# klkuhlm/unconfined

Hardware: AMD Instinct MI355X
Metric: (t,r) drawdown points/sec, Neuman-1974 1024x256 sweep; max |rel err| vs CPU ref (higher is better)
Workload: dtype f64

## Files before the change

unconfined_amd/csrc/ucf_device.h:

```cpp

#include "ucf_math.h"
#include "ucf_plan.h"
#include <cstdlib>

namespace UCF_NS {

using namespace ucfm;

#define UCF_STR_(x) #x
#define UCF_STR(x) UCF_STR_(x)
#define UCF_PI 3.14159265358979323846
#define UCF_EPS 2.220446049250313e-16

UCF_DEV double shfl_down1(double v) { return __shfl_down(v, 1, 64); }
UCF_DEV double shift_down1(double x)
{
    const int lo = __double2loint(x), hi = __double2hiint(x);
    const int l2 = __builtin_amdgcn_update_dpp(lo, lo, 0x130, 0xf, 0xf, false);
    const int h2 = __builtin_amdgcn_update_dpp(hi, hi, 0x130, 0xf, 0xf, false);
    return __hiloint2double(h2, l2);
}
UCF_DEV cplx shfl_down1(cplx v) { return cmake(shift_down1(v.re), shift_down1(v.im)); }
UCF_DEV cplx bcast0(cplx v) { return cmake(__shfl(v.re, 0, 64), __shfl(v.im, 0, 64)); }
UCF_DEV double wave_max(double v)
// ... 1245 lines not shown
__global__ void __launch_bounds__(UCF_WAVE * UCF_IWPB, WAVES)
integrate_kernel(const ucf_dev_params P0, int npts, int per_point, int nr, int nsv, int svmin,
                 const double* __restrict__ tDv, const double* __restrict__ rDv, const int* __restrict__ svv,
                 const double2* __restrict__ tab, int nt, int ir0, double2* __restrict__ state, int* __restrict__ ndone,
                 int* __restrict__ todo, const ucf_dev_params* __restrict__ Pv, int ppp, int pbase, int lsplit,
                 const double2* __restrict__ ltab, int nrows, int nheadw, int nworkw, int* __restrict__ wcount)
{
    extern __shared__ lds_c lds[];
#ifdef UCF_K1_ASSUME
    const ucf_dev_params& P = P0;
    UCF_K1_ASSUME
#endif
    const int lane = threadIdx.x & (UCF_WAVE - 1), wv = __builtin_amdgcn_readfirstlane(threadIdx.x / UCF_WAVE);
    constexpr int EF = (FAMILY == 5) ? 1 : FAMILY;
    constexpr bool ZPAIR = FOLD && EF == 2 && NZC == 1;
    const int nz = NZC ? NZC : P0.nz, R = P0.R, nacc = P0.nacc, N = P0.N, ngl = P0.ngl;
    __builtin_assume(nz >= 1 && R >= 1 && nacc >= 1 && ngl >= 1);
    const int nabs = N + nacc * ngl;
    {
        const double2* __restrict__ gt = (const double2*)P0.sc_tab;
        for (int k = threadIdx.x; k < UCF_SC_ENTRIES; k += UCF_WAVE * UCF_IWPB) lds[k] = gt[k];
    }
    __syncthreads();
    const lds_c* sct = lds;
    const int lslots = (NZC ? R : R + 1) * nz;
    lds_c* const wlds = lds + UCF_SC_ENTRIES + (size_t)wv * lslots * UCF_WAVE;
    lds_c* accTS = wlds;
    lds_c* accCur = wlds + (size_t)R * nz * UCF_WAVE;
    int ustat = blockIdx.x * UCF_IWPB + wv - gridDim.x * UCF_IWPB;
    auto next_unit = [&]() {
        if (!wcount) return ustat += gridDim.x * UCF_IWPB;
        int u = 0;
        if (lane == 0) u = __hip_atomic_fetch_add(wcount, 1, __ATOMIC_RELAXED, __HIP_MEMORY_SCOPE_AGENT);
        return __builtin_amdgcn_readfirstlane(u);
    };
    for (int wi = next_unit(); wi < nworkw; wi = next_unit()) {
        const bool tail = wi >= nheadw;
        const int ls = tail ? (lsplit >> 8) : (lsplit & 255), nsplit = 1 << ls;
        const int wj = tail ? wi - nheadw : wi;
        const int pt = (tail ? (nheadw >> (lsplit & 255)) : 0) + (wj >> ls), sub = wj & (nsplit - 1);
        auto part_bound = [&](int k) {
            if (k <= 0) return 0;
            if (k >= nsplit) return nabs;
            int j = (k * nabs / nsplit - N + ngl / 2) / ngl;
            j = j < 0 ? 0 : (j > nacc ? nacc : j);
            return N + j * ngl;
        };
        const int n0 = part_bound(sub), n1 = part_bound(sub + 1);
        if (n1 <= n0 && sub != 0) continue;
#ifdef UCF_TIMELINE
        const unsigned long long tl_t0 = __builtin_amdgcn_s_memtime();
#endif
        const work_item W = decode_item<LAYOUT>(P0, pt, lane, per_point, nr, nt, ir0, npts);
        const ucf_dev_params& P = item_params<MULTI>(P0, Pv, (LAYOUT == 3 ? W.plan * ppp : W.pidx) + pbase, ppp);
        bool need_lay1 = false, need_lay3 = false, need_lay12 = false;
        for (int z = 0; z < nz; z++) { need_lay1 |= (P.zLay[z] == 1); need_lay3 |= (P.zLay[z] == 3); need_lay12 |= (P.zLay[z] != 3); }
        const double tD = tDv[W.it], rD = rDv[W.ir];
        const int sv = (LAYOUT == 1) ? svmin : svv[W.it];
        const double2* __restrict__ row = tab + (size_t)(per_point ? W.pidx : (W.ir * nsv + (sv - svmin))) * nabs;
        const double tee = 2.0 * tD;
        const double sigma = P.alpha - P.logtol / (2.0 * tee);
        const cplx p = cmake(sigma, UCF_PI * W.mlap / tee);
        const double2 ltv = ltab[(size_t)(W.mlap < P0.np ? W.mlap : P0.np - 1) * nrows + W.it];
        const cplx lt = cmake(ltv.x, ltv.y);
        const lane_consts LC = make_lane_consts(P, p, lt);
        auto lt_again = [&]() {
            int it = W.it;
            asm volatile("" : "+v"(it));
            const double2 v = ltab[(size_t)(W.mlap < P0.np ? W.mlap : P0.np - 1) * nrows + it];
            return cmake(v.x, v.y);
        };
        double2* __restrict__ sti = state + (size_t)pt * state_slots(P0) * UCF_WAVE;
        double2* __restrict__ areas = sti + (size_t)(R + 1) * nz * UCF_WAVE;
        for (int s = 0; s < lslots; s++) lds_st(wlds, s, lane, cmake(0.0, 0.0));
        fast_common F;
        sc_ctx_init(F.sc, sct, UCF_KV(FAMILY, FOLD));
        const bool lane_ok = FAMILY != 2 || (fabs(LC.xifac.re) + fabs(LC.xifac.im) < 1.0e90);
        const int nlim = (__builtin_amdgcn_ballot_w64(!lane_ok) == 0) ? n1 : n0;

        int n = n0;
        double2 aa = row[n0 < nabs ? n0 : 0];
        int m = 0, jj = n0 > N ? (n0 - N) / ngl : 0;
        cplx acc0 = cmake(0.0, 0.0), acc1 = cmake(0.0, 0.0);
        if constexpr (ZPAIR) {
            int stopped = 0;
            const int nts = nlim < N ? nlim : N;
            for (; n < nts; n++) {
                const double2 nxt = row[n + 1 < nabs ? n + 1 : n];
                F.sc.salt = n;
                if (!fast_eta_wave<EF, true>(P, LC, aa.x, F)) { stopped = 1; break; }
                const cplx val = rscale(aa.y, fast_sample_zpair<!MULTI>(P, LC, F));
                const int n1 = n + 1;
                int tz = __builtin_ctz(n1);
                if (tz > R - 1) tz = R - 1;
                for (int sh = 0; sh <= tz; sh++) {
                    const int j = R - sh;
                    const double wl = P.ts_w[(size_t)(j - 1) * N + ((n1 >> sh) - 1)];
                    lds_st(accTS, j - 1, lane, cadd(lds_ld(accTS, j - 1, lane), rscale(wl, val)));
                }
                aa = nxt;
            }
            if (!stopped) for (; n < nlim; n++) {
                const double2 nxt = row[n + 1 < nabs ? n + 1 : n];
                F.sc.salt = n;
                if (!fast_eta_wave<EF, true>(P, LC, aa.x, F)) break;
                const cplx fz = fast_sample_zpair<!MULTI>(P, LC, F);
                acc0 = cmake(__builtin_fma(fz.re, aa.y, acc0.re), __builtin_fma(fz.im, aa.y, acc0.im));
                if (++m == ngl) {
                    const double lob = P.j0z[sv + jj - 1] / rD;
                    const double hib = P.j0z[sv + jj] / rD;
                    const double hw = (hib - lob) / 2.0;
                    const cplx ar = cmul(rscale(hw, acc0), lt_again());
                    areas[(size_t)jj * UCF_WAVE + lane] = make_double2(ar.re, ar.im);
                    acc0 = cmake(0.0, 0.0);
                    m = 0;
                    jj++;
                }
                aa = nxt;
            }
        } else
        for (; n < nlim; n++) {
            const double2 nxt = row[n + 1 < nabs ? n + 1 : n];
            const bool ts = n < N;
            F.sc.salt = n;
            if (!fast_eta_wave<EF, ZPAIR>(P, LC, aa.x, F)) break;
            if constexpr (!ZPAIR) fast_common_terms<EF, FOLD, LAY3, LAY1, NOFOLD, ZPAIR>(P, LC, aa.x, need_lay1, F, need_lay3, need_lay12);
            const int n1 = n + 1;
            int tz = __builtin_ctz(n1);
            if (tz > R - 1) tz = R - 1;
            for (int z = 0; z < nz; z++) {
                cplx fz;
                if constexpr (ZPAIR) fz = fast_sample_zpair<!MULTI>(P, LC, F);
                else fz = fast_sample_z<EF, FOLD, LAY3, LAY1, NOFOLD, ZPAIR>(P, F, z);
                if (ts) {
                    const cplx val = rscale(aa.y, fz);
                    for (int sh = 0; sh <= tz; sh++) {
                        const int j = R - sh;
                        const double wl = P.ts_w[(size_t)(j - 1) * N + ((n1 >> sh) - 1)];
                        const int slot = (j - 1) * nz + z;
                        lds_st(accTS, slot, lane, cadd(lds_ld(accTS, slot, lane), rscale(wl, val)));
                    }
                } else if (nz == 1 || (NZC == 2 && z == 0)) {
                    acc0 = cmake(__builtin_fma(fz.re, aa.y, acc0.re), __builtin_fma(fz.im, aa.y, acc0.im));
                } else if (NZC == 2) {
                    acc1 = cmake(__builtin_fma(fz.re, aa.y, acc1.re), __builtin_fma(fz.im, aa.y, acc1.im));
                } else {
                    const cplx a1 = lds_ld(accCur, z, lane);
                    lds_st(accCur, z, lane, cmake(__builtin_fma(fz.re, aa.y, a1.re), __builtin_fma(fz.im, aa.y, a1.im)));
                }
            }
            if (!ts && ++m == ngl) {
                const double lob = P.j0z[sv + jj - 1] / rD;
                const double hib = P.j0z[sv + jj] / rD;
                const double hw = (hib - lob) / 2.0;
                for (int z = 0; z < nz; z++) {
                    const cplx run = (nz == 1 || (NZC == 2 && z == 0)) ? acc0 : (NZC == 2 ? acc1 : lds_ld(accCur, z, lane));
                    const cplx ar = cmul(rscale(hw, run), lt);
                    areas[(size_t)(jj * nz + z) * UCF_WAVE + lane] = make_double2(ar.re, ar.im);
                    if (nz != 1 && NZC != 2) lds_st(accCur, z, lane, cmake(0.0, 0.0));
                }
                acc0 = acc1 = cmake(0.0, 0.0);
                m = 0;
                jj++;
            }
            aa = nxt;
        }
        if (sub == 0) {
            const cplx lte = ZPAIR ? lt_again() : lt;
            for (int s = 0; s < R * nz; s++) {
                const cplx v = cmul(lds_ld(wlds, s, lane), lte);
                sti[(size_t)s * UCF_WAVE + lane] = make_double2(v.re, v.im);
            }
            for (int s = R * nz; s < (R + 1) * nz; s++) sti[(size_t)s * UCF_WAVE + lane] = make_double2(0.0, 0.0);
        }
#ifdef UCF_TIMELINE
        if (sub == 0) {
            const unsigned long long tl_t1 = __builtin_amdgcn_s_memtime();
            const unsigned hwid = __builtin_amdgcn_s_getreg(63492);
            if (lane == 0) sti[(size_t)(R * nz) * UCF_WAVE + 0] = make_double2(__longlong_as_double((long long)tl_t0), __longlong_as_double((long long)tl_t1));
            if (lane == 1) sti[(size_t)(R * nz) * UCF_WAVE + 1] = make_double2((double)hwid, (double)__builtin_amdgcn_s_getreg(63508));
        }
#endif
        if (n < n1 && lane == 0) {
            const int nrep = (n < N) ? n : n - m;
            if (atomicMin(&ndone[pt], nrep) == nabs) todo[1 + atomicAdd(&todo[0], 1)] = pt;
        }
    }
}

#endif

template <int FAMILY, int LAYOUT>
__global__ void __launch_bounds__(UCF_WAVE, 3)
integrate_generic_kernel(const ucf_dev_params P, int npts, int per_point, int nr, int nsv, int svmin,
                         const double* __restrict__ tDv, const double* __restrict__ rDv, const int* __restrict__ svv,
                         const double2* __restrict__ tab, int nt, int ir0, double2* __restrict__ state, int* __restrict__ ndone)
{
    extern __shared__ lds_c lds[];
    const int lane = threadIdx.x;
    const int nz = P.nz, R = P.R, nacc = P.nacc, N = P.N, ngl = P.ngl;
    const int nabs = N + nacc * ngl;
    lds_c* accTS = lds;
    lds_c* accCur = lds + (size_t)R * nz * UCF_WAVE;
    lds_c* fdbuf = accCur + (size_t)nz * UCF_WAVE;
    bool need_lay1 = false;
    for (int z = 0; z < nz; z++) need_lay1 |= (P.zLay[z] == 1);
    for (int pt = blockIdx.x; pt < npts; pt += gridDim.x) {
        const work_item W = decode_item<LAYOUT>(P, pt, lane, per_point, nr, nt, ir0, npts);
        const double tD = tDv[W.it], rD = rDv[W.ir];
        const int sv = (LAYOUT == 1) ? svmin : svv[W.it];
        const double2* __restrict__ row = tab + (size_t)(per_point ? W.pidx : (W.ir * nsv + (sv - svmin))) * nabs;
        const double tee = 2.0 * tD;
        const double sigma = P.alpha - P.logtol / (2.0 * tee);
        const cplx p = cmake(sigma, UCF_PI * W.mlap / tee);
        const cplx lt = lap_time(P, p);
// ... 888 lines not shown
```

unconfined_amd/csrc/ucf_fastpath.h:

```cpp
#pragma once

namespace UCF_NS {

#define UCF_UNIFORM_BLOCK() asm volatile("" ::: "memory")
#define UCF_UNIFORM_BLOCK_F(FAMILY) do { if constexpr ((FAMILY) != 4) UCF_UNIFORM_BLOCK(); } while (0)

struct fprim {
    double ch, sh, ei, sn, cs;
};

template <bool POS>
UCF_DEV fprim prim_from_e(double x, double ax, double e, double ei, double y, const sc_ctx& sc)
{
    const int salt = sc.salt;
    fprim f;
    f.ei = ei;
    const double he = 0.5 * e;
    f.ch = __builtin_fma(0.5, ei, he);
    double s;
    if (ax < 0.35) {
        const double x2 = ax * ax;
        double pl = addk(mulk(x2, UCF_KHERE(1.0 / 6227020800.0, salt)), UCF_KHERE(1.0 / 39916800.0, salt));
        pl = fmak(pl, x2, UCF_KHERE(1.0 / 362880.0, salt));
        pl = fmak(pl, x2, UCF_KHERE(1.0 / 5040.0, salt));
        pl = fmak(pl, x2, UCF_KHERE(1.0 / 120.0, salt));
        pl = fmak(pl, x2, UCF_KHERE(1.0 / 6.0, salt));
        s = __builtin_fma(ax * x2, pl, ax);
    } else {
        s = __builtin_fma(-0.5, ei, he);
    }
    f.sh = POS ? s : copysign(s, x);
    sincos_tab_(y, sc, &f.sn, &f.cs);
    return f;
}
template <bool POS = false>
UCF_DEV fprim prim(double x, double y, const sc_ctx& sc)
{
    const double ax = POS ? x : fabs(x);
    const double e = exp_tab_(ax, sc);
    return prim_from_e<POS>(x, ax, e, fast_rcp(e), y, sc);
}
UCF_DEV void prim_pair(double x, double y, double zD, double xcap, const sc_ctx& sc, fprim* f, fprim* fz)
{
    const double xc = fmin(x, xcap);
    const double xz = xc * zD;
    const double e = exp_tab_(xc, sc), ez = exp_tab_(xz, sc);
    const double r = fast_rcp(e * ez);
    *f = prim_from_e<true>(xc, xc, e, r * ez, y, sc);
    *fz = prim_from_e<true>(xz, xz, ez, r * e, y * zD, sc);
}
template <bool UNI>
UCF_DEV void prim_pair_min(double x, double y, double zD, double xcap, const sc_ctx& sc, fprim* f, fprim* fz)
{
    double xc;
    if constexpr (UNI) asm("v_min_f64 %0, %1, %2" : "=v"(xc) : "v"(x), "s"(xcap));
    else xc = fmin(x, xcap);
    const double xz = xc * zD;
    const double e = exp_tab_(xc, sc), ez = exp_tab_(xz, sc);
    const double r = fast_rcp(e * ez);
    *f = prim_from_e<true>(xc, xc, e, r * ez, y, sc);
    *fz = prim_from_e<true>(xz, xz, ez, r * e, y * zD, sc);
}
UCF_DEV fprim prim_difference(const fprim& a, const fprim& b)
{
    fprim f;
    const double e = (a.ch + a.sh) * b.ei;
    const double ei = a.ei * (b.ch + b.sh);
    f.ei = ei;
    f.ch = 0.5 * (e + ei);
    f.sh = 0.5 * (e - ei);
    f.sn = __builtin_fma(a.sn, b.cs, -(a.cs * b.sn));
    f.cs = __builtin_fma(a.cs, b.cs, a.sn * b.sn);
    return f;
}
UCF_DEV cplx pcosh(const fprim& f) { return cmake(f.ch * f.cs, f.sh * f.sn); }
UCF_DEV cplx psinh(const fprim& f) { return cmake(f.sh * f.cs, f.ch * f.sn); }
UCF_DEV cplx pexpneg(const fprim& f) { return cmake(f.ei * f.cs, -(f.ei * f.sn)); }

UCF_DEV cplx expneg_direct(double x, double y, const sc_ctx& sc)
{
    const double ei = exp_tab_(-x, sc);
    double sn, cs;
    sincos_tab_(y, sc, &sn, &cs);
    return cmake(ei * cs, -(ei * sn));
}

UCF_DEV cplx cfma(cplx a, cplx b, cplx c)
{
    return cmake(__builtin_fma(a.re, b.re, __builtin_fma(-a.im, b.im, c.re)), __builtin_fma(a.re, b.im, __builtin_fma(a.im, b.re, c.im)));
}
UCF_DEV cplx cfnma(cplx a, cplx b, cplx c)
{
    return cmake(__builtin_fma(-a.re, b.re, __builtin_fma(a.im, b.im, c.re)), __builtin_fma(-a.re, b.im, __builtin_fma(-a.im, b.re, c.im)));
}
UCF_DEV cplx cinv_plain(cplx z)
{
    const double r = fast_rcp(z.re * z.re + z.im * z.im);
    return cmake(z.re * r, -(z.im * r));
}
UCF_DEV cplx cinv_scaled(cplx z)
{
    const double m = fmax(fabs(z.re), fabs(z.im));
    const int il = __builtin_amdgcn_frexp_exp(m) - 1;
    const double c = ldexp(z.re, -il), d = ldexp(z.im, -il);
    const double r = fast_rcp(c * c + d * d);
    return cmake(ldexp(c * r, -il), ldexp(-(d * r), -il));
}

UCF_DEV cplx cinv_auto(cplx z)
{
    const double m = fmax(fabs(z.re), fabs(z.im));
    if (__builtin_amdgcn_ballot_w64(!(m < 1.0e150 && m > 1.0e-150)) == 0) return cinv_plain(z);
    return cinv_scaled(z);
}

struct lane_consts {
    cplx p, lt, xifac;
    cplx fdB1;
    cplx mnpv;
};

UCF_DEV lane_consts make_lane_consts(const ucf_dev_params& P, cplx p, cplx lt)
{
    lane_consts L;
    L.p = p;
    L.lt = lt;
    cplx xf = rscale(P.alphaD, cinv_plain(p));
    if (P.model == 3) {
        cplx sum = cmake(0.0, 0.0);
        for (int j = 0; j < P.MoenchM; j++) sum = cadd(sum, cinv_plain(radd(1.0, cscale(p, P.MoenchInvGamma[j]))));
        xf = cmul(cscale(xf, (double)P.MoenchM), cinv_plain(sum));
    }
    L.xifac = xf;
    L.fdB1 = cscale(cscale(cscale(p, P.fd_beta0), P.fd_expmb2), P.inv_kappa);
    L.mnpv = radd(1.0, cscale(p, P.mn_vartheta * P.mn_c3));
    return L;
}

struct fast_common {
    sc_ctx sc;
    cplx th, eta, ff1, ff2, inv_she, she, che, top, g3, inv_den, ex1;
    cplx chz0;
    fprim p1;
    int have_p1;
    cplx mn_uod;
#ifdef UCF_SINGLE_RCP
    cplx q, den;
#endif
    cplx fd_s1;
    cplx top3, fd_s13;
    bool small_eta, fd_use, fd_use3;
    int any_small, any_large;
};

template <int FAMILY>
UCF_DEV double fast_scale(const ucf_dev_params& P)
{
    if (FAMILY == 0 || FAMILY == 3) return 2.0;
    if (FAMILY == 5) return P.inv_bD;
    return (FAMILY == 2 && P.model == 4) ? 2.0 : 2.0 * P.inv_bD;
}

template <int FAMILY, bool PAIR = false>
UCF_DEV bool fast_eta(const ucf_dev_params& P, const lane_consts& L, double a, fast_common& S)
{
    const double a2 = a * a;
    const cplx q = caddr(L.p, a2);
#ifdef UCF_SINGLE_RCP
    S.q = q;
#endif
    double mq = 0.0;
    if (PAIR && FAMILY != 0) {
        double r;
        rsq_pair(q.re * q.re + q.im * q.im, &mq, &r);
        S.th = cmake(q.re * r, -(q.im * r));
    } else {
        const double r = fast_rcp(q.re * q.re + q.im * q.im);
        S.th = cmake(q.re * r, -(q.im * r));
    }
    if (FAMILY == 0) return q.re > 0.0;
    {
        const double qr = q.re * P.inv_kappa, qi = q.im * P.inv_kappa;
        double r, hr;
        const double d = PAIR ? mq * P.inv_kappa : sqrt_only(__builtin_fma(qr, qr, qi * qi));
        sqrt_hrsqrt(0.5 * (d + qr), &r, &hr);
        S.eta = cmake(r, qi * hr);
    }
    return (S.eta.re <= P.fast_eta_max) & (q.re > 0.0) & (fabs(S.eta.im) < P.fast_im_max);
}
template <int FAMILY, bool PAIR = false>
UCF_DEV bool fast_eta_wave(const ucf_dev_params& P, const lane_consts& L, double a, fast_common& S)
{
    (void)fast_eta<FAMILY, PAIR>(P, L, a, S);
    const cplx q = caddr(L.p, a * a);
    unsigned long long bad = __builtin_amdgcn_ballot_w64(!(q.re > 0.0));
    if (FAMILY != 0) {
        bad |= __builtin_amdgcn_ballot_w64(!(S.eta.re <= P.fast_eta_max));
        bad |= __builtin_amdgcn_ballot_w64(!(fabs(S.eta.im) < P.fast_im_max));
    }
    return bad == 0;
}

template <int FAMILY, bool FOLD = false, bool LAY3 = true, bool LAY1 = true, bool NOFOLD = false, bool ZPAIR = false>
UCF_DEV void fast_common_terms(const ucf_dev_params& P, const lane_consts& L, double a, bool need_lay1_in, fast_common& S,
                               bool need_lay3_in = false, bool need_lay12 = true)
{
    static_assert(!ZPAIR || (FOLD && FAMILY == 2), "ZPAIR: folded water-table kernels only");
    const double a2 = a * a;
    if (FAMILY == 0) return;
    if (FAMILY == 3) {
        const fprim p1 = prim<true>(S.eta.re, S.eta.im, S.sc);
        S.che = pcosh(p1);
        S.she = psinh(p1);
        const double wr = __builtin_fma(a2, P.mn_c3, L.mnpv.re), wi = L.mnpv.im;
        double vr, hr;
        sqrt_hrsqrt(0.5 * (sqrt_only(__builtin_fma(wr, wr, wi * wi)) + wr), &vr, &hr);
        const cplx u = cmake(P.mn_u0 * (1.0 - vr), -(P.mn_u0 * (wi * hr)));
        const cplx Delta0 = cfnma(u, S.che, cmul(S.eta, S.she));
        S.mn_uod = cmul(u, cinv_auto(Delta0));
        return;
    }
    const bool hantush = NOFOLD || !(FAMILY == 2 && P.model == 4);
    const bool z1 = FOLD || (!NOFOLD && P.fold_dD != 0), z2 = FOLD || (!NOFOLD && P.fold_lD1 != 0);
    const bool need_lay1 = (FOLD || !LAY1) ? false : need_lay1_in;
    const bool need_lay3 = (FOLD || !LAY3) ? false : need_lay3_in;
    S.small_eta = (FAMILY != 2) || (S.eta.re < P.maxexp);
    S.any_small = ((FAMILY != 2) || (__builtin_amdgcn_ballot_w64(S.small_eta) != 0)) ? 1 : 0;
    S.any_large = ((FAMILY == 2) && (__builtin_amdgcn_ballot_w64(!S.small_eta) != 0)) ? 1 : 0;
    const bool need_p1 = (hantush && (!(z1 && z2) || need_lay1)) || FAMILY == 4 || (FAMILY == 2 && S.any_small);
    S.have_p1 = (need_p1 && !z2) ? 1 : 0;
    fprim p1;
    if (ZPAIR && need_p1) {
        fprim pz;
        prim_pair(S.eta.re, S.eta.im, P.zD[0], P.maxexp, S.sc, &p1, &pz);
        S.chz0 = pcosh(pz);
        S.che = pcosh(p1);
        S.she = psinh(p1);
        S.ex1 = cmake(0.0, 0.0);
    } else if (need_p1) {
        p1 = prim<true>(S.eta.re, S.eta.im, S.sc);
        if (!z2) S.p1 = p1;
        S.che = pcosh(p1);
        S.she = psinh(p1);
        if (need_lay1) S.ex1 = pexpneg(p1);
        else S.ex1 = cmake(0.0, 0.0);
    } else {
        S.che = S.she = S.ex1 = cmake(0.0, 0.0);
    }
    if (hantush) {
        fprim pd;
        if (!z1) { pd = prim<true>(S.eta.re * P.dD, S.eta.im * P.dD, S.sc); S.ff1 = psinh(pd); }
        else S.ff1 = cmake(0.0, 0.0);
        fprim pl;
        if (!z2) { pl = prim<true>(S.eta.re * P.lD1, S.eta.im * P.lD1, S.sc); S.ff2 = psinh(pl); }
        else S.ff2 = cmake(0.0, 0.0);
        if (!(z1 && z2) || need_lay1) S.inv_she = cinv_auto(S.she);
        if (need_lay1) {
            const cplx exl = z2 ? cmake(1.0, 0.0) : pexpneg(pl);
            S.g3 = csub(exl, cmul(cadd(S.ff1, cmul(S.ex1, S.ff2)), S.inv_she));
        }
        if (FAMILY != 1) {
            S.top = S.top3 = S.th;
            if (!(z1 && z2)) {
                if (need_lay12) {
                    cplx g1;
                    if (z1) g1 = cmake(1.0, 0.0);
                    else if (P.share_g1top == 1) g1 = pcosh(pd);
                    else if (P.share_g1top == 2) g1 = csub(pcosh(pd), cmul(rscale(P.g1_delta, S.eta), S.ff1));
                    else { const double c = P.dD1 - 1.0; g1 = pcosh(prim(S.eta.re * c, S.eta.im * c, S.sc)); }
                    const cplx udp = csub(g1, cmul(cadd(cmul(S.ff1, S.che), S.ff2), S.inv_she));
                    S.top = cmul(udp, S.th);
                }
                if (need_lay3) {
                    cplx sd1 = S.she;
                    if (!z1) {
                        const double x1 = S.eta.re * P.dD1;
                        if (__builtin_amdgcn_ballot_w64(!(x1 >= 1.0)) == 0) sd1 = psinh(prim_difference(p1, pd));
                        else sd1 = psinh(prim(x1, S.eta.im * P.dD1, S.sc));
                    }
                    const cplx udp = cmul(z2 ? sd1 : csub(sd1, S.ff2), S.inv_she);
                    S.top3 = cmul(udp, S.th);
// ... 75 lines not shown
    cplx chz = cmake(1.0, 0.0);
    fprim pz;
    if (ZPAIR) { if (need_chz) chz = S.chz0; }
    else if (need_chz) { pz = prim<true>(S.eta.re * zD, S.eta.im * zD, S.sc); chz = pcosh(pz); }
    *chz_out = chz;
    cplx udp;
    if (lay == 1) {
        udp = cmul(S.g3, chz);
    } else {
        cplx g2 = cmake(0.0, 0.0);
        const bool need_1z = !z2;
        fprim p1z;
        if (z2 && FAMILY == 2 && S.any_large) {
            const double c = 1.0 - zD;
            *exz_out = expneg_direct(S.eta.re * c, S.eta.im * c, S.sc);
            UCF_UNIFORM_BLOCK_F(FAMILY);
        }
        if (need_1z) {
            if (need_chz && S.have_p1 && zD >= 0.0 && zD <= 1.0) p1z = prim_difference(S.p1, pz);
            else
            { const double c = 1.0 - zD; p1z = prim(S.eta.re * c, S.eta.im * c, S.sc); }
        }
        if (!z2 && FAMILY == 2 && S.any_large) { *exz_out = pexpneg(p1z); UCF_UNIFORM_BLOCK_F(FAMILY); }
        cplx f2c = cmake(0.0, 0.0);
        if (!z2) f2c = cmul(S.ff2, pcosh(p1z));
        if (lay == 2 || !LAY3) {
            if (z1 && z2) { UCF_UNIFORM_BLOCK_F(FAMILY); return S.th; }
            cplx num = f2c;
            if (!z1) { num = cadd(cmul(S.ff1, chz), f2c); UCF_UNIFORM_BLOCK_F(FAMILY); }
            g2 = cmul(num, S.inv_she);
            udp = rsub(1.0, g2);
            UCF_UNIFORM_BLOCK_F(FAMILY);
        } else {
            const double ca = 2.0 - zD - P.dD, cb = zD - P.dD;
            const cplx sa = psinh(prim(S.eta.re * ca, S.eta.im * ca, S.sc));
            const cplx sb = psinh(prim(S.eta.re * cb, S.eta.im * cb, S.sc));
            const cplx num = cmake(__builtin_fma(0.5, sa.re + sb.re, -f2c.re), __builtin_fma(0.5, sa.im + sb.im, -f2c.im));
            udp = cmul(num, S.inv_she);
        }
    }
    const cplx res = cmul(udp, S.th);
    UCF_UNIFORM_BLOCK_F(FAMILY);
    return res;
}

template <int FAMILY, bool FOLD = false, bool LAY3 = true, bool LAY1 = true, bool NOFOLD = false, bool ZPAIR = false>
UCF_DEV cplx fast_sample_z(const ucf_dev_params& P, const fast_common& S, int iz)
{
    const double zD = P.zD[iz];
    const int lay = P.zLay[iz];
    cplx chz, exz = cmake(0.0, 0.0);
    if (FAMILY == 0) return S.th;
    if (FAMILY == 3) {
        const cplx cz = pcosh(prim<true>(S.eta.re * zD, S.eta.im * zD, S.sc));
        return cfma(S.th, cmul(S.mn_uod, cz), S.th);
    }
    if (FAMILY == 1) return fast_hantush_z<1, FOLD, LAY3, LAY1, NOFOLD>(P, S, zD, lay, &chz, &exz);
    if (FAMILY == 4) {
        const cplx sH = fast_hantush_z<4, FOLD, LAY3, LAY1, NOFOLD>(P, S, zD, lay, &chz, &exz);
        if (!FOLD && LAY3 && lay == 3) return S.fd_use3 ? cadd(sH, cmul(S.fd_s13, chz)) : sH;
        return S.fd_use ? cadd(sH, cmul(S.fd_s1, chz)) : sH;
    }
    cplx u;
    if (!NOFOLD && P.model == 4) {
        u = S.th;
        if (S.any_small) chz = ZPAIR ? S.chz0 : pcosh(prim(S.eta.re * zD, S.eta.im * zD, S.sc));
        if (S.any_large) { const double c = 1.0 - zD; exz = expneg_direct(S.eta.re * c, S.eta.im * c, S.sc); }
    } else {
        u = fast_hantush_z<2, FOLD, LAY3, LAY1, NOFOLD, ZPAIR>(P, S, zD, lay, &chz, &exz);
        if (LAY1 && S.any_large && lay == 1) { const double c = 1.0 - zD; exz = expneg_direct(S.eta.re * c, S.eta.im * c, S.sc); }
    }
#ifdef UCF_SINGLE_RCP
    if (FOLD || (!NOFOLD && P.model == 4)) return cmul(csub(S.den, S.small_eta ? chz : exz), S.inv_den);
#endif
    const cplx top = (!FOLD && LAY3 && (NOFOLD || P.model != 4) && lay == 3) ? S.top3 : S.top;
    cplx g = chz;
    if (S.any_large) {
        g = S.small_eta ? chz : exz;
        asm volatile("" ::: "memory");
    }
    return cfnma(cmul(top, g), S.inv_den, u);
}

template <bool UNI>
UCF_DEV cplx fast_sample_zpair(const ucf_dev_params& P, const lane_consts& L, const fast_common& S)
{
    const double zD = P.zD[0];
    const bool small_eta = S.eta.re < P.maxexp;
    const bool any_small = __builtin_amdgcn_ballot_w64(small_eta) != 0, any_large = __builtin_amdgcn_ballot_w64(!small_eta) != 0;
    cplx den, g;
    if (!any_large) {
        fprim p1, pz;
        prim_pair_min<UNI>(S.eta.re, S.eta.im, zD, P.maxexp, S.sc, &p1, &pz);
        g = pcosh(pz);
        const cplx che = pcosh(p1), she = psinh(p1);
        const cplx xi = cmul(S.eta, L.xifac);
        if (P.beta != 0.0) den = cfma(radd(1.0, cmul(rscale(P.beta, S.eta), xi)), che, cmul(xi, she));
        else den = cfma(xi, she, che);
        UCF_UNIFORM_BLOCK();
    } else if (!any_small) {
        const double c = 1.0 - zD;
        g = expneg_direct(S.eta.re * c, S.eta.im * c, S.sc);
        const cplx xi = cmul(S.eta, L.xifac);
        if (P.beta != 0.0) den = cadd(radd(1.0, cmul(rscale(P.beta, S.eta), xi)), xi);
        else den = radd(1.0, xi);
        UCF_UNIFORM_BLOCK();
    } else {
        fprim p1, pz;
        prim_pair_min<UNI>(S.eta.re, S.eta.im, zD, P.maxexp, S.sc, &p1, &pz);
        const cplx chz = pcosh(pz), che = pcosh(p1), she = psinh(p1);
        const cplx xi = cmul(S.eta, L.xifac);
        if (P.beta != 0.0) {
            const cplx one_bex = radd(1.0, cmul(rscale(P.beta, S.eta), xi));
            den = small_eta ? cfma(one_bex, che, cmul(xi, she)) : cadd(one_bex, xi);
        } else {
            den = small_eta ? cfma(xi, she, che) : radd(1.0, xi);
        }
        const double c = 1.0 - zD;
        const cplx exz = expneg_direct(S.eta.re * c, S.eta.im * c, S.sc);
        g = small_eta ? chz : exz;
        UCF_UNIFORM_BLOCK();
    }
    const double r = fast_rcp(__builtin_fma(den.im, den.im, den.re * den.re));
    const cplx inv_den = cmake(den.re * r, -(den.im * r));
    return cfnma(cmul(S.th, g), inv_den, S.th);
}


}
```

unconfined_amd/csrc/ucf_math.h:

```cpp
#include <hip/hip_runtime.h>
#include <math.h>

#ifndef UCF_FAST
#define UCF_FAST 0
#endif

#define UCF_DEV __device__ __forceinline__

#ifndef UCF_NS
#error "define UCF_NS (ucf_faithful / ucf_fast) before including ucf_math.h"
#endif
namespace UCF_NS {
namespace ucfm {

struct cplx {
    double re, im;
};

UCF_DEV cplx cmake(double re, double im) { cplx z; z.re = re; z.im = im; return z; }
UCF_DEV cplx cadd(cplx a, cplx b) { return cmake(a.re + b.re, a.im + b.im); }
UCF_DEV cplx csub(cplx a, cplx b) { return cmake(a.re - b.re, a.im - b.im); }
UCF_DEV cplx cneg(cplx a) { return cmake(-a.re, -a.im); }
#if UCF_FAST
UCF_DEV cplx cmul(cplx a, cplx b)
// ... 140 lines not shown

UCF_DEV double cabs_(cplx z) { return hypot(z.re, z.im); }
UCF_DEV bool c_is_finite(cplx z)
{
    if (d_isnan(z.re) || d_isnan(z.im)) return false;
    const double m = fmax(fabs(z.re), fabs(z.im));
    if (__builtin_expect(m < 1.2e308, 1)) return true;
    const double h = cabs_(z);
    return !(h > 1.7976931348623157e308);
}
UCF_DEV bool c_abs_positive(cplx z)
{
    const bool inf = d_isinf(z.re) || d_isinf(z.im);
    const bool nan = d_isnan(z.re) || d_isnan(z.im);
    return inf || (!nan && (z.re != 0.0 || z.im != 0.0));
}

#define UCF_T709 709
#define UCF_DBL_MIN 2.2250738585072014e-308
#define UCF_DBL_MAX 1.7976931348623157e308

#if UCF_FAST
__device__ __noinline__ static double2 sincos_huge_(double y) { double s, c; sincos(y, &s, &c); return make_double2(s, c); }

UCF_DEV void sincos_medium_(double x, double* sn, double* cs)
{
    const int salt = __builtin_amdgcn_readfirstlane(__double2hiint(x));
#define K(c) UCF_KHERE(c, salt)
    const double fn = __builtin_rint(mulk(x, K(6.36619772367581382433e-01)));
    const double r = __builtin_fma(-fn, 1.57079632673412561417e+00, x);
    const double w = mulk(fn, K(6.07710050650619224932e-11));
    const double y0 = r - w;
    const double y1 = (r - y0) - w;
    const double z = y0 * y0;
    const double v = z * y0;
    const double rs = fmak(z, fmak(z, fmak(z, addk(mulk(z, K(1.58969099521155010221e-10)), K(-2.50507602534068634195e-08)),
                                           K(2.75573137070700676789e-06)), K(-1.98412698298579493134e-04)), K(8.33333333332248946124e-03));
    const double ksin = y0 - ((z * (0.5 * y1 - v * rs) - y1) - mulk(v, K(-1.66666666666666324348e-01)));
    const double ww = z * z;
    const double rc = __builtin_fma(ww * ww, fmak(z, addk(mulk(z, K(-1.13596475577881948265e-11)), K(2.08757232129817482790e-09)), K(-2.75573143513906633035e-07)),
                                    z * fmak(z, addk(mulk(z, K(2.48015872894767294178e-05)), K(-1.38888888888741095749e-03)), K(4.16666666666666019037e-02)));
#undef K
    const double hz = 0.5 * z;
    const double w1 = 1.0 - hz;
    const double kcos = w1 + (((1.0 - w1) - hz) + (z * rc - y0 * y1));
    const int q = (int)fn & 3;
    const double s_sel = (q & 1) ? kcos : ksin;
    const double c_sel = (q & 1) ? ksin : kcos;
    *sn = (q & 2) ? -s_sel : s_sel;
    *cs = ((q + 1) & 2) ? -c_sel : c_sel;
}
#define UCF_SC_N 256
struct sc_ctx {
    const double2* tab;
    int salt;
    int kv;
    double magic, s7, c6, e5;
};
#define UCF_MAGIC 6755399441055744.0
UCF_DEV void sc_ctx_init(sc_ctx& C, const double2* tab, int kv)
{
    C.tab = tab;
    C.salt = 0;
    C.kv = kv;
    C.magic = UCF_MAGIC;
    C.s7 = -1.98412698412698412698e-04;
    C.c6 = -1.38888888888888888889e-03;
    C.e5 = 1.0 / 120.0;
    if (kv >= 1) asm volatile("" : "+v"(C.magic));
    if (kv >= 4) asm volatile("" : "+v"(C.s7), "+v"(C.c6), "+v"(C.e5));
}
UCF_DEV double fma_vsv(double a, double c, double b)
{
    double o;
    asm("v_fma_f64 %0, %1, %2, %3" : "=v"(o) : "v"(a), "s"(c), "v"(b));
    return o;
}
#define UCF_SC_MAGIC_ADD(t, fn, x, c, C, salt)                                                           \
    double t, fn;                                                                                        \
    if ((C).kv >= 1) { t = fma_vsv(x, c, (C).magic); fn = t - (C).magic; }                               \
    else { t = addk(mulk(x, c), UCF_KHERE(UCF_MAGIC, salt)); fn = addk(t, UCF_KHERE(-UCF_MAGIC, salt)); }
#define UCF_SC_LEAD(z, av, a, b, C, salt) (((C).kv >= 4) ? fmak(z, av, UCF_KHERE(b, salt)) : addk(mulk(z, UCF_KHERE(a, salt)), UCF_KHERE(b, salt)))

UCF_DEV void sincos_tab_(double x, const sc_ctx& C, double* sn, double* cs)
{
    const int salt = C.salt;
#define K(c) UCF_KHERE(c, salt)
    UCF_SC_MAGIC_ADD(t, fn, x, K(4.07436654315252059568e+01), C, salt)
    const int k = __double2loint(t) & (UCF_SC_N - 1);
    const double r = __builtin_fma(-fn, 2.45436926052207127214e-02, x);
    const double y = __builtin_fma(-fn, 9.49546954141592538956e-13, r);
    const double2 T = C.tab[k];
    const double z = y * y;
    const double ps = fmak(z, UCF_SC_LEAD(z, C.s7, -1.98412698412698412698e-04, 8.33333333333333333333e-03, C, salt), K(-1.66666666666666666667e-01));
    const double pc = fmak(z, UCF_SC_LEAD(z, C.c6, -1.38888888888888888889e-03, 4.16666666666666666667e-02, C, salt), K(-0.5));
#undef K
    const double sy = __builtin_fma(y * z, ps, y);
    const double cm1 = z * pc;
    *sn = T.x + __builtin_fma(T.x, cm1, T.y * sy);
    *cs = T.y + __builtin_fma(T.y, cm1, -(T.x * sy));
}

#define UCF_EX_N 128
UCF_DEV double exp_tab_(double x, const sc_ctx& C)
{
    const int salt = C.salt;
#define K(c) UCF_KHERE(c, salt)
    UCF_SC_MAGIC_ADD(t, fn, x, K(184.6649652337873161420704), C, salt)
    const int k = __double2loint(t);
    double r = __builtin_fma(-fn, 0x1.62e42feep-8, x);
    r = __builtin_fma(-fn, 1.4907929134926466e-12, r);
    const double2 T = C.tab[UCF_SC_N + (k & (UCF_EX_N - 1))];
    double q = UCF_SC_LEAD(r, C.e5, 1.0 / 120.0, 1.0 / 24.0, C, salt);
    q = fmak(q, r, K(1.0 / 6.0));
#undef K
    q = __builtin_fma(q, r, 0.5);
    const double p = __builtin_fma(r * r, q, r);
    return ldexp(T.x + __builtin_fma(T.x, p, T.y), k >> 7);
}

UCF_DEV void sincos_(double x, double* sn, double* cs)
{
    if (__builtin_expect(!(fabs(x) < 1.0e6), 0)) {
        const double2 sc = sincos_huge_(x);
        *sn = sc.x;
        *cs = sc.y;
        return;
    }
    sincos_medium_(x, sn, cs);
}
#else
__device__ __noinline__ static double2 sincos_libm_(double y) { double s, c; sincos(y, &s, &c); return make_double2(s, c); }
UCF_DEV void sincos_(double y, double* s, double* c)
{
    if (fabs(y) > UCF_DBL_MIN) {
        const double2 sc = sincos_libm_(y);
        *s = sc.x;
        *c = sc.y;
    } else {
        *s = y;
        *c = 1.0;
    }
}
__device__ __noinline__ static double2 coshsinh_libm_(double x) { return make_double2(cosh(x), sinh(x)); }
#endif

UCF_DEV void coshsinh_(double x, double* ch, double* sh)
{
#if UCF_FAST
    const double ax = fabs(x);
    const double e = exp(ax);
    const double ei = fast_rcp(e);
    *ch = 0.5 * (e + ei);
    double s;
    if (ax < 0.35) {
        const double x2 = ax * ax;
        double pl = 1.0 / 355687428096000.0;
        pl = pl * x2 + 1.0 / 1307674368000.0;
        pl = pl * x2 + 1.0 / 6227020800.0;
        pl = pl * x2 + 1.0 / 39916800.0;
        pl = pl * x2 + 1.0 / 362880.0;
        pl = pl * x2 + 1.0 / 5040.0;
        pl = pl * x2 + 1.0 / 120.0;
        pl = pl * x2 + 1.0 / 6.0;
        s = ax + ax * (x2 * pl);
    } else {
// ... 179 lines not shown
```

Before: 8.585 million.

## Add phase-latched wave-uniform fast paths for z-pair sampling loop

Adds per-wave phase flags for the z-pair Hankel integration loop. Once a wave-wide check proves that eta stays in range, that imaginary parts are small, or that every lane is in the large-eta regime, later iterations skip the matching ballots and branch selection. When all lanes have a tiny argument, it also swaps the table-based sincos for a short Taylor polynomial with no table lookup. This is meant to cut per-iteration validation and transcendental cost, at the price of extra code paths and the assumption that these monotonic regime properties keep holding as the abscissa grows.

```diff
diff --git a/unconfined_amd/csrc/ucf_device.h b/unconfined_amd/csrc/ucf_device.h
--- a/unconfined_amd/csrc/ucf_device.h
+++ b/unconfined_amd/csrc/ucf_device.h
@@ -1351,14 +1351,18 @@
         double2 aa = row[n0 < nabs ? n0 : 0];
         int m = 0, jj = n0 > N ? (n0 - N) / ngl : 0;
         cplx acc0 = cmake(0.0, 0.0), acc1 = cmake(0.0, 0.0);
+        int zph = 0;
         if constexpr (ZPAIR) {
             int stopped = 0;
+            zph = 0;
+            if (!MULTI && nlim > n0)
+                zph = zpair_part_phase(P, LC, P.j0z[sv - 1 + (nlim > N ? (nlim - N + ngl - 1) / ngl : 0)] / rD);
             const int nts = nlim < N ? nlim : N;
             for (; n < nts; n++) {
                 const double2 nxt = row[n + 1 < nabs ? n + 1 : n];
                 F.sc.salt = n;
-                if (!fast_eta_wave<EF, true>(P, LC, aa.x, F)) { stopped = 1; break; }
-                const cplx val = rscale(aa.y, fast_sample_zpair<!MULTI>(P, LC, F));
+                if (!fast_eta_wave_zpair<!MULTI>(P, LC, aa.x, F, zph, 1)) { stopped = 1; break; }
+                const cplx val = rscale(aa.y, fast_sample_zpair<!MULTI>(P, LC, F, zph, 1));
                 const int n1 = n + 1;
                 int tz = __builtin_ctz(n1);
                 if (tz > R - 1) tz = R - 1;
@@ -1372,8 +1376,9 @@
             if (!stopped) for (; n < nlim; n++) {
                 const double2 nxt = row[n + 1 < nabs ? n + 1 : n];
                 F.sc.salt = n;
-                if (!fast_eta_wave<EF, true>(P, LC, aa.x, F)) break;
-                const cplx fz = fast_sample_zpair<!MULTI>(P, LC, F);
+                const int last = m == ngl - 1;
+                if (!fast_eta_wave_zpair<!MULTI>(P, LC, aa.x, F, zph, last)) break;
+                const cplx fz = fast_sample_zpair<!MULTI>(P, LC, F, zph, last);
                 acc0 = cmake(__builtin_fma(fz.re, aa.y, acc0.re), __builtin_fma(fz.im, aa.y, acc0.im));
                 if (++m == ngl) {
                     const double lob = P.j0z[sv + jj - 1] / rD;
@@ -1399,7 +1404,7 @@
             if (tz > R - 1) tz = R - 1;
             for (int z = 0; z < nz; z++) {
                 cplx fz;
-                if constexpr (ZPAIR) fz = fast_sample_zpair<!MULTI>(P, LC, F);
+                if constexpr (ZPAIR) fz = fast_sample_zpair<!MULTI>(P, LC, F, zph, 0);
                 else fz = fast_sample_z<EF, FOLD, LAY3, LAY1, NOFOLD, ZPAIR>(P, F, z);
                 if (ts) {
                     const cplx val = rscale(aa.y, fz);
diff --git a/unconfined_amd/csrc/ucf_fastpath.h b/unconfined_amd/csrc/ucf_fastpath.h
--- a/unconfined_amd/csrc/ucf_fastpath.h
+++ b/unconfined_amd/csrc/ucf_fastpath.h
@@ -9,7 +9,7 @@
     double ch, sh, ei, sn, cs;
 };
 
-template <bool POS>
+template <bool POS, bool SMALLY = false>
 UCF_DEV fprim prim_from_e(double x, double ax, double e, double ei, double y, const sc_ctx& sc)
 {
     const int salt = sc.salt;
@@ -30,7 +30,8 @@
         s = __builtin_fma(-0.5, ei, he);
     }
     f.sh = POS ? s : copysign(s, x);
-    sincos_tab_(y, sc, &f.sn, &f.cs);
+    if (SMALLY) sincos_small_(y, sc, &f.sn, &f.cs);
+    else sincos_tab_(y, sc, &f.sn, &f.cs);
     return f;
 }
 template <bool POS = false>
@@ -83,6 +84,24 @@
     double sn, cs;
     sincos_tab_(y, sc, &sn, &cs);
     return cmake(ei * cs, -(ei * sn));
+}
+
+UCF_DEV cplx expneg_small(double x, double y, const sc_ctx& sc)
+{
+    const double ei = exp_tab_(-x, sc);
+    double sn, cs;
+    sincos_small_(y, sc, &sn, &cs);
+    return cmake(ei * cs, -(ei * sn));
+}
+UCF_DEV void prim_pair_small(double x, double y, double zD, double xcap, const sc_ctx& sc, fprim* f, fprim* fz)
+{
+    double xc;
+    asm("v_min_f64 %0, %1, %2" : "=v"(xc) : "v"(x), "s"(xcap));
+    const double xz = xc * zD;
+    const double e = exp_tab_(xc, sc), ez = exp_tab_(xz, sc);
+    const double r = fast_rcp(e * ez);
+    *f = prim_from_e<true, true>(xc, xc, e, r * ez, y, sc);
+    *fz = prim_from_e<true, true>(xz, xz, ez, r * e, y * zD, sc);
 }
 
 UCF_DEV cplx cfma(cplx a, cplx b, cplx c)
@@ -197,6 +216,44 @@
     if (FAMILY != 0) {
         bad |= __builtin_amdgcn_ballot_w64(!(S.eta.re <= P.fast_eta_max));
         bad |= __builtin_amdgcn_ballot_w64(!(fabs(S.eta.im) < P.fast_im_max));
+    }
+    return bad == 0;
+}
+
+#ifndef UCF_ZPAIR_PHASES
+#define UCF_ZPAIR_PHASES 3
+#endif
+enum {
+    UCF_PH_RANGE = 1,
+    UCF_PH_IM = 2,
+    UCF_PH_LARGE = 4,
+    UCF_PH_YS = 8,
+    UCF_PH_YL = 16
+};
+UCF_DEV int zpair_part_phase(const ucf_dev_params& P, const lane_consts& L, double a_max)
+{
+    if (!(UCF_ZPAIR_PHASES & 2)) return 0;
+    const double lim = 0.99 * P.fast_eta_max;
+    const bool ok = (L.p.re > 0.0) & (lim > 0.0) & ((__builtin_fma(a_max, a_max, fabs(L.p.re) + fabs(L.p.im)) * P.inv_kappa) < lim * lim);
+    return __builtin_amdgcn_ballot_w64(!ok) == 0 ? UCF_PH_RANGE : 0;
+}
+template <bool UNI>
+UCF_DEV bool fast_eta_wave_zpair(const ucf_dev_params& P, const lane_consts& L, double a, fast_common& S, int& ph, int may_set)
+{
+    if constexpr (!UNI) return fast_eta_wave<2, true>(P, L, a, S);
+    (void)fast_eta<2, true>(P, L, a, S);
+    unsigned long long bad = 0;
+    if (!(ph & UCF_PH_RANGE)) {
+        const cplx q = caddr(L.p, a * a);
+        bad |= __builtin_amdgcn_ballot_w64(!(q.re > 0.0));
+        bad |= __builtin_amdgcn_ballot_w64(!(S.eta.re <= P.fast_eta_max));
+        UCF_UNIFORM_BLOCK();
+    }
+    if (!(ph & UCF_PH_IM)) {
+        const double ai = fabs(S.eta.im);
+        bad |= __builtin_amdgcn_ballot_w64(!(ai < P.fast_im_max));
+        if ((UCF_ZPAIR_PHASES & 2) && may_set && __builtin_amdgcn_ballot_w64(!(ai < 0.5 * P.fast_im_max)) == 0) ph |= UCF_PH_IM;
+        UCF_UNIFORM_BLOCK();
     }
     return bad == 0;
 }
@@ -438,30 +495,68 @@
     return cfnma(cmul(top, g), S.inv_den, u);
 }
 
+template <bool UNI, bool SMALLY>
+UCF_DEV void zpair_arm_small(const ucf_dev_params& P, const lane_consts& L, const fast_common& S, double zD, cplx* g, cplx* den)
+{
+    fprim p1, pz;
+    if (SMALLY) prim_pair_small(S.eta.re, S.eta.im, zD, P.maxexp, S.sc, &p1, &pz);
+    else prim_pair_min<UNI>(S.eta.re, S.eta.im, zD, P.maxexp, S.sc, &p1, &pz);
+    *g = pcosh(pz);
+    const cplx che = pcosh(p1), she = psinh(p1);
+    const cplx xi = cmul(S.eta, L.xifac);
+    if (P.beta != 0.0) *den = cfma(radd(1.0, cmul(rscale(P.beta, S.eta), xi)), che, cmul(xi, she));
+    else *den = cfma(xi, she, che);
+}
+template <bool SMALLY>
+UCF_DEV void zpair_arm_large(const ucf_dev_params& P, const lane_consts& L, const fast_common& S, double x, double y, cplx* g, cplx* den)
+{
+    *g = SMALLY ? expneg_small(x, y, S.sc) : expneg_direct(x, y, S.sc);
+    const cplx xi = cmul(S.eta, L.xifac);
+    if (P.beta != 0.0) *den = cadd(radd(1.0, cmul(rscale(P.beta, S.eta), xi)), xi);
+    else *den = radd(1.0, xi);
+}
 template <bool UNI>
-UCF_DEV cplx fast_sample_zpair(const ucf_dev_params& P, const lane_consts& L, const fast_common& S)
-{
+UCF_DEV cplx fast_sample_zpair(const ucf_dev_params& P, const lane_consts& L, const fast_common& S, int& ph, int may_set)
+{
+    constexpr bool SHORT = UNI && (UCF_ZPAIR_PHASES & 1);
     const double zD = P.zD[0];
-    const bool small_eta = S.eta.re < P.maxexp;
-    const bool any_small = __builtin_amdgcn_ballot_w64(small_eta) != 0, any_large = __builtin_amdgcn_ballot_w64(!small_eta) != 0;
+    int form = 2;
+    if (!UNI || !(ph & UCF_PH_LARGE)) {
+        const bool small_eta = S.eta.re < P.maxexp;
+        const bool any_small = __builtin_amdgcn_ballot_w64(small_eta) != 0, any_large = __builtin_amdgcn_ballot_w64(!small_eta) != 0;
+        form = !any_large ? 0 : (any_small ? 1 : 2);
+        if (UNI && (UCF_ZPAIR_PHASES & 2) && may_set && form == 2 && __builtin_amdgcn_ballot_w64(!(S.eta.re > P.maxexp * (1.0 + 0x1p-20))) == 0) ph |= UCF_PH_LARGE;
+        UCF_UNIFORM_BLOCK();
+    }
     cplx den, g;
-    if (!any_large) {
-        fprim p1, pz;
-        prim_pair_min<UNI>(S.eta.re, S.eta.im, zD, P.maxexp, S.sc, &p1, &pz);
-        g = pcosh(pz);
-        const cplx che = pcosh(p1), she = psinh(p1);
-        const cplx xi = cmul(S.eta, L.xifac);
-        if (P.beta != 0.0) den = cfma(radd(1.0, cmul(rscale(P.beta, S.eta), xi)), che, cmul(xi, she));
-        else den = cfma(xi, she, che);
-        UCF_UNIFORM_BLOCK();
-    } else if (!any_small) {
+    if (form == 0) {
+        if (SHORT && may_set && !(ph & UCF_PH_YS)) {
+            if (__builtin_amdgcn_ballot_w64(!(fabs(S.eta.im) < UCF_SC_SMALL)) == 0) ph |= UCF_PH_YS | UCF_PH_YL;
+            UCF_UNIFORM_BLOCK();
+        }
+        if (SHORT && (ph & UCF_PH_YS)) {
+            zpair_arm_small<UNI, true>(P, L, S, zD, &g, &den);
+            UCF_UNIFORM_BLOCK();
+        } else {
+            zpair_arm_small<UNI, false>(P, L, S, zD, &g, &den);
+            UCF_UNIFORM_BLOCK();
+        }
+    } else if (form == 2) {
         const double c = 1.0 - zD;
-        g = expneg_direct(S.eta.re * c, S.eta.im * c, S.sc);
-        const cplx xi = cmul(S.eta, L.xifac);
-        if (P.beta != 0.0) den = cadd(radd(1.0, cmul(rscale(P.beta, S.eta), xi)), xi);
-        else den = radd(1.0, xi);
-        UCF_UNIFORM_BLOCK();
-    } else {
+        const double x = S.eta.re * c, y = S.eta.im * c;
+        if (SHORT && may_set && !(ph & UCF_PH_YL)) {
+            if (__builtin_amdgcn_ballot_w64(!(fabs(y) < UCF_SC_SMALL)) == 0) ph |= UCF_PH_YL;
+            UCF_UNIFORM_BLOCK();
+        }
+        if (SHORT && (ph & UCF_PH_YL)) {
+            zpair_arm_large<true>(P, L, S, x, y, &g, &den);
+            UCF_UNIFORM_BLOCK();
+        } else {
+            zpair_arm_large<false>(P, L, S, x, y, &g, &den);
+            UCF_UNIFORM_BLOCK();
+        }
+    } else {
+        const bool small_eta = S.eta.re < P.maxexp;
         fprim p1, pz;
         prim_pair_min<UNI>(S.eta.re, S.eta.im, zD, P.maxexp, S.sc, &p1, &pz);
         const cplx chz = pcosh(pz), che = pcosh(p1), she = psinh(p1);
diff --git a/unconfined_amd/csrc/ucf_math.h b/unconfined_amd/csrc/ucf_math.h
--- a/unconfined_amd/csrc/ucf_math.h
+++ b/unconfined_amd/csrc/ucf_math.h
@@ -246,6 +246,21 @@
     else { t = addk(mulk(x, c), UCF_KHERE(UCF_MAGIC, salt)); fn = addk(t, UCF_KHERE(-UCF_MAGIC, salt)); }
 #define UCF_SC_LEAD(z, av, a, b, C, salt) (((C).kv >= 4) ? fmak(z, av, UCF_KHERE(b, salt)) : addk(mulk(z, UCF_KHERE(a, salt)), UCF_KHERE(b, salt)))
 
+#define UCF_SC_SMALL 0.012
+UCF_DEV void sincos_small_(double y, const sc_ctx& C, double* sn, double* cs)
+{
+    const int salt = C.salt;
+#define K(c) UCF_KHERE(c, salt)
+    const double z = y * y;
+    const double ps = fmak(z, UCF_SC_LEAD(z, C.s7, -1.98412698412698412698e-04, 8.33333333333333333333e-03, C, salt), K(-1.66666666666666666667e-01));
+    const double pc = fmak(z, UCF_SC_LEAD(z, C.c6, -1.38888888888888888889e-03, 4.16666666666666666667e-02, C, salt), K(-0.5));
+#undef K
+    double cm1 = z * pc;
+    asm("" : "+v"(cm1));
+    *sn = __builtin_fma(y * z, ps, y);
+    *cs = 1.0 + cm1;
+}
+
 UCF_DEV void sincos_tab_(double x, const sc_ctx& C, double* sn, double* cs)
 {
     const int salt = C.salt;
```

After: 8.994 million, median of 6. +4.8%, better.
